# AcrylicShrimp/omok-ai

Hardware: NVIDIA B200
Metric: mcts_simulations_per_sec (higher is better)
Workload: dtype f32

## Files before the change

omok-ai_b200/csrc/omk_api.cu:

```cuda
#include <cstdio>
#include <cstdlib>
#include <cstring>
#include <string>
#include <vector>

#include <utility>

#include "omk_internal.h"

using namespace omk;

static thread_local std::string g_err;
static int32_t fail(int32_t code, const std::string &msg) {
    g_err = msg;
    return code;
}
#define CK(call)                                                                                        \
    do {                                                                                                \
        cudaError_t e__ = (call);                                                                       \
        if (e__ != cudaSuccess)                                                                         \
            return fail(OMK_ERR_CUDA, std::string(#call) + ": " + cudaGetErrorString(e__));             \
    } while (0)
#define CKV(call)                                                                                       \
    do {                                                                                                \
// ... 30 lines not shown
#define SCRATCH(i, count, ptr)                          \
    do {                                                \
        int32_t rc__ = scratch_dev(c, (i), (count), &(ptr)); \
        if (rc__) return rc__;                          \
    } while (0)

static int32_t ensure_workspace(omk_ctx *c, int rows) {
    rows = (rows + 255) / 256 * 256;
    Workspace &w = c->ws;
    if (rows <= w.max_rows) return OMK_OK;
    const size_t r = (size_t)rows;
    w.max_rows = 0;
    CK(w.nn_in.grow(c->stream, r));
    CK(w.req_tree.grow(c->stream, r));
    CK(w.req_node.grow(c->stream, r));
    CK(w.P.grow(c->stream, r * kRow));
    CK(w.V.grow(c->stream, r));
    CK(cudaMemsetAsync(w.nn_in, 0, w.nn_in.bytes(), c->stream));
    w.max_rows = rows;
    return OMK_OK;
}

namespace omk {
bool ensure_activations(omk_ctx *c, int rows) {
    Workspace &w = c->ws;
    rows = (rows + 255) / 256 * 256;
    const bool want_fp32 = c->tower_mode == 0 || c->fc0_mode == 0;
    if (rows <= w.act_rows && (!want_fp32 || w.act_fp32)) return true;
    if (rows < w.act_rows) rows = w.act_rows;
    if (cudaStreamSynchronize(c->stream) != cudaSuccess) return false;
// ... 281 lines not shown
    if (out_h2d) *out_h2d = c->h2d_bytes;
    if (out_d2h) *out_d2h = c->d2h_bytes;
    return OMK_OK;
}

static int32_t sp_refresh_root_policy(omk_ctx *c);

extern "C" int32_t omk_net_load_params(omk_ctx *c, const float *const *tensors, const int64_t *lens) {
    CK(cudaSetDevice(c->device));
    for (int i = 0; i < kNetTensors; ++i)
        if (!tensors[i] || lens[i] != kLens[i])
            return fail(OMK_ERR_INVALID, "tensor " + std::to_string(i) + ": expected " + std::to_string(kLens[i]) + " elements");
    for (int i = 0; i < kNetTensors; ++i)
        CK(copy_h2d(c, c->net.t[i], tensors[i], sizeof(float) * (size_t)kLens[i], c->stream));
    c->net_pack_dirty = false;
    net_pack_heads(c);
    if (!fc16_prepare_weights(c)) return fail(OMK_ERR_CUDA, "fp16-split fc weight preparation failed");
    if (!tower16_prepare_weights(c)) return fail(OMK_ERR_CUDA, "fp16-split tower weight preparation failed");
    CK(cudaStreamSynchronize(c->stream));
    c->net.loaded = true;
    return sp_refresh_root_policy(c);
}
extern "C" int32_t omk_net_get_params(omk_ctx *c, float *const *tensors, const int64_t *lens) {
    CK(cudaSetDevice(c->device));
    if (!c->net.loaded) return fail(OMK_ERR_STATE, "network weights not loaded");
    for (int i = 0; i < kNetTensors; ++i)
        if (!tensors[i] || lens[i] != kLens[i]) return fail(OMK_ERR_INVALID, "bad tensor length");
    for (int i = 0; i < kNetTensors; ++i)
        CK(copy_d2h(c, tensors[i], c->net.t[i], sizeof(float) * (size_t)kLens[i], c->stream));
    CK(cudaStreamSynchronize(c->stream));
    return OMK_OK;
}
extern "C" int32_t omk_net_init_random(omk_ctx *c, uint64_t seed) {
    CK(cudaSetDevice(c->device));
    launch_net_init_random(c, seed);
    c->net_pack_dirty = false;
    net_pack_heads(c);
    if (!fc16_prepare_weights(c)) return fail(OMK_ERR_CUDA, "fp16-split fc weight preparation failed");
    if (!tower16_prepare_weights(c)) return fail(OMK_ERR_CUDA, "fp16-split tower weight preparation failed");
    CK(cudaStreamSynchronize(c->stream));
    CK(cudaGetLastError());
    c->net.loaded = true;
    return sp_refresh_root_policy(c);
}

static int32_t net_eval_common(omk_ctx *c, int n, const float *images_dev, float *out_p, float *out_v, int slot = 0) {
    if (slot == 0) {
        int32_t rc_p = ensure_packed(c);
        if (rc_p) return rc_p;
    }
    ModelScope scope(c, slot);
// ... 35 lines not shown
    CK(cudaSetDevice(c->device));
    if (!c->net.loaded) return fail(OMK_ERR_STATE, "network weights not loaded");
    if (n < 0 || !images || !out_p) return fail(OMK_ERR_INVALID, "bad arguments");
    if (n == 0) return OMK_OK;
    int32_t rc = ensure_workspace(c, n);
    if (rc) return rc;
    float *d_img = nullptr;
    SCRATCH(0, (size_t)n * 243, d_img);
    CK(copy_h2d(c, d_img, images, sizeof(float) * (size_t)n * 243, c->stream));
    const uint32_t nn = (uint32_t)n;
    CK(copy_h2d(c, c->ws.n_req, &nn, sizeof nn, c->stream));
    return net_eval_common(c, n, d_img, out_p, out_v);
}

static int32_t weights_changed(omk_ctx *c) {
    net_pack_heads(c);
    if (!fc16_prepare_weights(c)) return fail(OMK_ERR_CUDA, "fp16-split fc weight preparation failed");
    if (!tower16_prepare_weights(c)) return fail(OMK_ERR_CUDA, "fp16-split tower weight preparation failed");
    CK(cudaStreamSynchronize(c->stream));
    return sp_refresh_root_policy(c);
}

static int32_t train_backward_impl(omk_ctx *c, const float *images, const float *pi, const float *z, int32_t n,
                                   void **out_grads_device, int64_t *out_count, bool sync) {
    CK(cudaSetDevice(c->device));
    if (!c->net.loaded) return fail(OMK_ERR_STATE, "network weights not loaded");
    if (n < 1 || !images || !pi || !z) return fail(OMK_ERR_INVALID, "bad arguments");
    float *g = nullptr;
    c->train_n = 0;
    if (const char *e = train_backward_step(c, images, pi, z, n, &g)) return fail(OMK_ERR_CUDA, std::string("omk_train_backward: ") + e);
// ... 60 lines not shown
extern "C" int32_t omk_train_comm_init(omk_ctx *c, const uint8_t *id, int32_t nranks, int32_t rank) {
    CK(cudaSetDevice(c->device));
    if (!id || nranks < 1 || rank < 0 || rank >= nranks) return fail(OMK_ERR_INVALID, "bad communicator arguments");
    if (const char *e = train_comm_init(c, id, nranks, rank)) return fail(OMK_ERR_STATE, std::string("NCCL: ") + e);
    return OMK_OK;
}
extern "C" int32_t omk_train_comm_destroy(omk_ctx *c) {
    CK(cudaSetDevice(c->device));
    train_comm_destroy(c);
    return OMK_OK;
}

extern "C" int32_t omk_debug_set_fc0_mode(omk_ctx *c, int32_t mode) {
    if (mode != 0 && mode != 1) return fail(OMK_ERR_INVALID, "fc0 mode must be 1 (tcgen05 3xFP16) or 0 (fp32 CUDA cores, A/B check)");
    c->fc0_mode = mode;
    return OMK_OK;
}
extern "C" int32_t omk_debug_set_tower_mode(omk_ctx *c, int32_t mode) {
    if (mode != 0 && mode != 1) return fail(OMK_ERR_INVALID, "tower mode must be 1 (tcgen05 3xFP16) or 0 (fp32 CUDA cores, A/B check)");
    c->tower_mode = mode;
    return OMK_OK;
}
extern "C" int32_t omk_debug_set_fc0_balance(omk_ctx *c, int32_t on) {
    if (on != 0 && on != 1) return fail(OMK_ERR_INVALID, "fc0 balance must be 0 or 1");
    c->fc0_balance = on;
    return OMK_OK;
}
extern "C" int32_t omk_debug_set_fc0_chunk(omk_ctx *c, int32_t k_blocks) {
    if (k_blocks != 3 && k_blocks != 9) return fail(OMK_ERR_INVALID, "fc0 chunk must be 9 (default) or 3 (finer accumulation)");
    CK(cudaStreamSynchronize(c->stream));
    c->fc0_chunk = k_blocks;
    return OMK_OK;
}
extern "C" int32_t omk_debug_set_lane_min_trees(omk_ctx *c, int32_t min_trees) {
    if (min_trees < 0) return fail(OMK_ERR_INVALID, "min_trees < 0");
    c->lane_min_trees = min_trees;
    return OMK_OK;
}
extern "C" int32_t omk_debug_tower_timing(omk_ctx *c, int64_t *out64) {
    CK(cudaSetDevice(c->device));
    CK(cudaStreamSynchronize(c->stream));
    tower16_read_timing(reinterpret_cast<long long *>(out64));
    return OMK_OK;
}
extern "C" int32_t omk_debug_get_buffer(omk_ctx *c, int32_t which, float *out, int64_t count) {
    CK(cudaSetDevice(c->device));
// ... 566 lines not shown
        int8_t *d_status = reinterpret_cast<int8_t *>(ds + slot.off_status);
        for (int l = 0; l < lanes; ++l) {
            LaneScope scope(c, l, 0);
            const int g0 = lane_g0[l], nl = lane_n[l];
            bool sp = span_begin(OMK_K_MOVE);
            launch_sp_prepare(c, g0, nl, mover, other, modes, temps);
            launch_root_noise(c, mover + g0, nl, cfg.epsilon, cfg.alpha);
            span_end(sp);
        }
        for (int r = 0; r < rounds; ++r) {
            for (int l = 0; l < lanes; ++l) {
                LaneScope scope(c, l, 0);
                const int g0 = lane_g0[l], nl = lane_n[l];
                bool sp = span_begin(OMK_K_SELECT);
                launch_reset_requests(c);
                launch_select_expand(c, mover + g0, nl, cfg.batch_size);
                span_end(sp);
                RUN_EVAL(c, cfg.evaluator, nl * cfg.batch_size);
                sp = span_begin(OMK_K_APPLY);
                launch_apply(c, mover + g0, nl, kApplySearch);
                span_end(sp);
            }
        }
        for (int l = 0; l < lanes; ++l) {
            LaneScope scope(c, l, 0);
            const int g0 = lane_g0[l], nl = lane_n[l];
            const size_t row = (size_t)g0;
            bool sp = span_begin(OMK_K_MOVE);
            launch_sample(c, mover + g0, nl, modes + g0, temps + g0, actions + g0, policy_out + (size_t)g0 * kCells, nullptr);
            launch_sp_record(c, nl, mover + g0, actions + g0, policy_out + (size_t)g0 * kCells, d_boards + row * kCells,
                             d_policy + row * kCells, d_actions + row);
            if (feed) {
                CK(cudaStreamWaitEvent(c->stream, c->rp.ev_commit, 0));
                launch_rp_stage(c, g0, nl, d_boards + row * kCells, d_policy + row * kCells);
            }
// ... 665 lines not shown
```

omok-ai_b200/csrc/omk_device.cuh:

```cuda
#pragma once
#include <cstdint>
#include <cuda_runtime.h>

namespace omk {

constexpr int kCells = 81;
constexpr int kSide = 9;
constexpr int kRow = 96;
constexpr uint32_t kNoNode = 0xFFFFu;
constexpr float kF32Eps = 1.1920929e-7f;

constexpr int kInProgress = 0, kDraw = 1, kBlackWin = 2, kWhiteWin = 3;

constexpr int kNodeBytes = 1408;
constexpr int kOffPolicy = 64;
constexpr int kOffEdgeN = 448;
constexpr int kOffEdgeW = 832;
constexpr int kOffChild = 1216;

struct NodeHdr {
    uint32_t black[3], white[3], cmask[3];
    uint32_t parent, action, status, legal, turn, has_policy;
};

struct __align__(16) TreeHdr {
    uint32_t n_nodes;
    uint32_t root_n;
    float root_w;
    float root_p;
    uint32_t rng_counter;
    uint32_t stream;
    uint32_t noise_epoch;
    uint32_t error;
    uint32_t sims_lo, sims_hi;
    uint32_t pad[6];
};
static_assert(sizeof(TreeHdr) == 64, "TreeHdr is 64 bytes");

// ... 13 lines not shown
    return tree_nodes + (size_t)id * kNodeBytes;
}
__device__ __forceinline__ float *node_policy(uint8_t *n) { return reinterpret_cast<float *>(n + kOffPolicy); }
__device__ __forceinline__ uint32_t *node_edge_n(uint8_t *n) { return reinterpret_cast<uint32_t *>(n + kOffEdgeN); }
__device__ __forceinline__ float *node_edge_w(uint8_t *n) { return reinterpret_cast<float *>(n + kOffEdgeW); }
__device__ __forceinline__ uint16_t *node_child(uint8_t *n) { return reinterpret_cast<uint16_t *>(n + kOffChild); }

__device__ __forceinline__ NodeHdr load_hdr(const uint8_t *n) {
    const uint4 *q = reinterpret_cast<const uint4 *>(n);
    const uint4 a = q[0], b = q[1], c = q[2];
    NodeHdr h;
    h.black[0] = a.x; h.black[1] = a.y; h.black[2] = a.z;
    h.white[0] = a.w; h.white[1] = b.x; h.white[2] = b.y;
    h.cmask[0] = b.z; h.cmask[1] = b.w; h.cmask[2] = c.x;
    h.parent = c.y & 0xFFFFu; h.action = (c.y >> 16) & 0xFFu; h.status = c.y >> 24;
    h.legal = c.z & 0xFFu; h.turn = (c.z >> 8) & 0xFFu; h.has_policy = (c.z >> 16) & 0xFFu;
    return h;
}
__device__ __forceinline__ void store_hdr(uint8_t *n, const NodeHdr &h) {
    uint4 *q = reinterpret_cast<uint4 *>(n);
    q[0] = make_uint4(h.black[0], h.black[1], h.black[2], h.white[0]);
    q[1] = make_uint4(h.white[1], h.white[2], h.cmask[0], h.cmask[1]);
    q[2] = make_uint4(h.cmask[2], h.parent | (h.action << 16) | (h.status << 24),
                      h.legal | (h.turn << 8) | (h.has_policy << 16), 0u);
}

__device__ __forceinline__ uint32_t sel3(uint32_t w0, uint32_t w1, uint32_t w2, int word) {
    return word == 0 ? w0 : (word == 1 ? w1 : w2);
}
__device__ __forceinline__ bool bit81(const uint32_t *m, int i) { return (sel3(m[0], m[1], m[2], i >> 5) >> (i & 31)) & 1u; }
__device__ __forceinline__ void set81(uint32_t *m, int i) {
    const uint32_t b = 1u << (i & 31);
    if ((i >> 5) == 0) m[0] |= b; else if ((i >> 5) == 1) m[1] |= b; else m[2] |= b;
}
__device__ __forceinline__ int popc81(const uint32_t *m) { return __popc(m[0]) + __popc(m[1]) + __popc(m[2] & 0x1FFFFu); }
__device__ __forceinline__ int nth_set_bit32(uint32_t w, int r) {
    for (int i = 0; i < r; ++i) w &= w - 1;
    return __ffs(w) - 1;
}
// ... 182 lines not shown
```

omok-ai_b200/csrc/omk_internal.h:

```cpp
#pragma once
#include <cstdint>
#include <memory>
#include <utility>
#include <vector>
#include <cuda.h>
#include <cuda_fp16.h>
#include <cuda_runtime.h>

#include "../../include/omok_b200.h"
#include "omk_device.cuh"

namespace omk {

constexpr int kMaxBatchPerTree = 64;
constexpr int kNetTensors = 31;
constexpr int kModelSlots = 16;

enum ApplyMode { kApplySearch = 0, kApplyNewGame = 1, kApplyEnsure = 2 };

struct DeviceMem {
    static cudaError_t alloc(void **p, size_t bytes) { return cudaMalloc(p, bytes); }
    static void release(void *p) { cudaFree(p); }
};
struct PinnedMem {
// ... 83 lines not shown
    bool act_fp32 = false;
    Buf<__half> act0_h16, act0_l16;
    Buf<__half> act1_h16, act1_l16;
    Buf<__half> act2_h16, act2_l16;
    Buf<float> act2;
    Buf<float> logits;
    Buf<float> act0;
    Buf<float> act1;
    ActMaps maps;
};
struct Workspace : Activations {
    int max_rows = 0;
    Buf<NNIn> nn_in;
    Buf<uint32_t> req_tree;
    Buf<uint32_t> req_node;
    Buf<float> P;
    Buf<float> V;
    Buf<uint32_t> n_req;
    Buf<uint32_t> slot_base, slot_count;
    Buf<int32_t> ids;
    Buf<int32_t> actions;
    Buf<uint8_t> modes;
    Buf<float> temps;
    Buf<int8_t> status;
    Buf<float> policy_out;
    Buf<uint32_t> streams;
    Buf<float> splitk_partial;
    Buf<float4> bal_partial;
    Buf<uint32_t> bal_flags;
};
// ... 73 lines not shown
    omk::NetWeights opp;
    omk::NetWeights more[omk::kModelSlots - 2];
    omk::NetWeights *model = &net;
    omk::NetWeights &slot(int s) { return s == 0 ? net : (s == 1 ? opp : more[s - 2]); }
    omk::Workspace ws;
    int virtual_loss = 0;
    int fc0_balance = 0;
    int fc0_chunk = 9;
    int fc0_mode = 1;
    std::unique_ptr<omk::Fc16State, omk::Fc16StateFree> fc16_state;
    int tower16_pairs = 0;
    std::unique_ptr<omk::TrainState, omk::TrainStateFree> train_state;
    int train_n = 0;
    bool net_pack_dirty = false;
    int tower_mode = 1;

    omk_selfplay_config sp_cfg{};
    bool sp_active = false;
    omk::Buf<int32_t> sp_ply;
    omk::Buf<uint8_t> sp_buf;
    static constexpr int kSpRing = 4;
    omk::Buf<uint8_t> sp_ring_dev;
    omk::PinnedBuf<uint8_t> sp_ring_host;
    size_t sp_ring_slot_bytes = 0;
    cudaStream_t sp_copy_stream = nullptr;
    cudaEvent_t sp_ev_rec[kSpRing][2] = {}, sp_ev_copy[kSpRing] = {};
    omk::Replay rp;
    omk::Buf<uint8_t> eval_buf;
    cudaEvent_t ev0 = nullptr, ev1 = nullptr;
};
// ... 1 lines not shown
namespace omk {

void launch_env_reset(omk_ctx *c, const int32_t *ids_dev, int n);
void launch_env_step(omk_ctx *c, const int32_t *ids_dev, const uint8_t *actions_dev, int n, int8_t *status_dev,
                     uint32_t *legal_dev);
void launch_env_get(omk_ctx *c, const int32_t *ids_dev, int n, uint8_t *boards_dev, uint8_t *turns_dev,
                    uint16_t *legal_dev);
void launch_env_set(omk_ctx *c, const int32_t *ids_dev, int n, const uint8_t *boards_dev, const uint8_t *turns_dev);
void launch_env_encode(omk_ctx *c, const int32_t *ids_dev, int n, int mode, float *out_dev);
void launch_env_playout(omk_ctx *c, int n, int plies, uint8_t *actions_dev, int8_t *status_dev);
void launch_pack_boards(omk_ctx *c, const uint8_t *boards_dev, const uint8_t *turns_dev, int n, int mode);

void launch_new_games(omk_ctx *c, const int32_t *ids_dev, int n, const uint32_t *streams_dev,
                      const int8_t *only_if_terminal, const float *root_policy);
void launch_root_noise(omk_ctx *c, const int32_t *ids_dev, int n, float epsilon, float alpha);
void launch_select_expand(omk_ctx *c, const int32_t *ids_dev, int n, int batch);
void launch_apply(omk_ctx *c, const int32_t *ids_dev, int n, int mode);
void launch_sample(omk_ctx *c, const int32_t *ids_dev, int n, const uint8_t *modes_dev, const float *temps_dev,
                   int32_t *actions_dev, float *policy_dev, uint8_t *valid_dev);
void launch_ensure_prepare(omk_ctx *c, const int32_t *ids_dev, const int32_t *actions_dev, int n);
void launch_play(omk_ctx *c, const int32_t *ids_dev, const int32_t *actions_dev, int n, int8_t *status_dev);
void launch_root_children(omk_ctx *c, int tree, int32_t *actions_dev, unsigned long long *n_dev, float *w_dev,
                          float *p_dev, int32_t *len_dev, float *policy_dev, uint32_t *misc_dev);
void launch_eval_hash(omk_ctx *c, int rows_bound);
void launch_pool_get_envs(omk_ctx *c, const int32_t *ids_dev, int n, uint8_t *boards_dev, uint8_t *turns_dev,
                          uint16_t *legal_dev, int8_t *status_dev);
void launch_reset_requests(omk_ctx *c);
void launch_sp_prepare(omk_ctx *c, int g0, int n, int32_t *mover, int32_t *other, uint8_t *modes, float *temps);
void launch_sp_record(omk_ctx *c, int n, const int32_t *mover, const int32_t *actions, const float *policy_in,
                      uint8_t *boards_out, float *policy_out, int32_t *actions_out);
void launch_sp_advance(omk_ctx *c, int g0, int n, const int8_t *status, unsigned long long *counters);

// ... 65 lines not shown
```

omok-ai_b200/csrc/tree_kernels.cu:

```cuda
#include "omk_internal.h"

namespace omk {

constexpr int kWarpsPerBlock = 4;
constexpr unsigned kFull = 0xffffffffu;

struct TreeArgs {
    TreeHdr *hdrs;
    uint8_t *nodes;
    int cap_nodes;
    const int32_t *ids;
    int id_base;
    int n;
    uint64_t seed;
    uint32_t *dev_error;
    unsigned long long *dev_sims;
    NNIn *nn_in;
    uint32_t *req_tree, *req_node;
    uint32_t *n_req;
    uint32_t *slot_base, *slot_count;
    const float *P, *V;
    int max_rows;
    int vloss;
};

__device__ __forceinline__ int tree_of(const TreeArgs &a, int slot) { return a.ids ? a.ids[slot] : slot + a.id_base; }
__device__ __forceinline__ uint8_t *tree_nodes_of(const TreeArgs &a, int tree) {
    return a.nodes + (size_t)tree * (size_t)a.cap_nodes * kNodeBytes;
}

__device__ __forceinline__ float dummy_prior(const NodeHdr &h, int a) {
    const uint32_t occ = sel3(h.black[0] | h.white[0], h.black[1] | h.white[1], h.black[2] | h.white[2], a >> 5);
    if ((occ >> (a & 31)) & 1u) return 0.0f;
    if (h.legal == 0) return 1.0f;
    return __fmul_rn(1.0f, __fdiv_rn(1.0f, (float)h.legal));
}

__device__ __forceinline__ float seq_sum81(const float v[3]) {
    float s = 0.0f;
#pragma unroll
    for (int j = 0; j < 3; ++j) {
        const int lim = j == 2 ? kCells - 64 : 32;
        for (int l = 0; l < lim; ++l) s = __fadd_rn(s, __shfl_sync(kFull, v[j], l));
// ... 104 lines not shown
        const float inv = __fdiv_rn(1.0f, s);
#pragma unroll
        for (int j = 0; j < 3; ++j) nz[j] = __fmul_rn(nz[j], inv);
        if (lane == 0) th->noise_epoch = epoch + 1;
    }
    const float keep = __fsub_rn(1.0f, epsilon);
#pragma unroll
    for (int j = 0; j < 3; ++j) p[j] = __fadd_rn(__fmul_rn(keep, p[j]), __fmul_rn(epsilon, nz[j]));
    const float s = seq_sum81(p);
    const float inv = __fdiv_rn(1.0f, s);
#pragma unroll
    for (int j = 0; j < 3; ++j) {
        const int c = lane + 32 * j;
        if (c < kCells) pol[c] = __fmul_rn(p[j], inv);
    }
    if (lane == 0 && !h.has_policy) {
        h.has_policy = 1;
        store_hdr(tn, h);
    }
}

__global__ void __launch_bounds__(kWarpsPerBlock * 32) k_select_expand(TreeArgs a, int batch) {
    __shared__ uint32_t s_path[kWarpsPerBlock][kCells + 3];
    __shared__ uint16_t s_req[kWarpsPerBlock][kMaxBatchPerTree];
    const int wib = threadIdx.x >> 5;
    const int slot = blockIdx.x * kWarpsPerBlock + wib;
    const int lane = threadIdx.x & 31;
    if (slot >= a.n) return;
    const int tree = tree_of(a, slot);
    uint8_t *tn = tree_nodes_of(a, tree);
    TreeHdr *th = &a.hdrs[tree];
    uint32_t *path = s_path[wib];
    uint16_t *req = s_req[wib];

    uint32_t n_nodes = th->n_nodes;
    uint32_t root_n = th->root_n;
    float root_w = th->root_w;
    uint32_t rng_counter = th->rng_counter;
    const uint32_t stream = th->stream;
    uint32_t err = th->error;
    uint32_t sims = 0;
    int nreq = 0;

    bool restart = true;
    uint32_t x = 0;
    uint32_t cur_n = root_n;
    int depth = 0;
    NodeHdr h{};
    int it = 0;
    while (it < batch && !err) {
        if (restart) {
            x = 0;
            cur_n = root_n;
            depth = 0;
            h = load_hdr(tn);
            restart = false;
        }
        for (;;) {
            const int nch = popc81(h.cmask);
            if (nch != (int)h.legal || nch == 0) break;
            uint8_t *xn = node_ptr(tn, x);
            const uint32_t parent_n = cur_n > 1u ? cur_n : 1u;
            const float sq = __fsqrt_rn((float)parent_n);
            const uint32_t *en = node_edge_n(xn);
            const float *ew = node_edge_w(xn);
            const float *pol = node_policy(xn);
            const uint16_t *ch = node_child(xn);
            unsigned long long best = 0ull;
            uint32_t best_n = 0;
            int best_a = 0;
// ... 18 lines not shown
            }
            unsigned long long wbest = best;
#pragma unroll
            for (int off = 16; off > 0; off >>= 1) {
                const unsigned long long o = __shfl_xor_sync(kFull, wbest, off);
                wbest = o > wbest ? o : wbest;
            }
            const int src = __ffs(__ballot_sync(kFull, best == wbest && best != 0ull)) - 1;
            best_n = __shfl_sync(kFull, best_n, src);
            best_a = __shfl_sync(kFull, best_a, src);
            if (lane == 0) path[depth] = (x << 8) | (uint32_t)best_a;
            ++depth;
            x = (uint32_t)(wbest & 0xFFFFFFFFull) - 1u;
            cur_n = best_n;
            h = load_hdr(node_ptr(tn, x));
        }
        __syncwarp();

        if (h.status != kInProgress) {
            ++it;
            ++sims;
            if (lane == 0) {
                const float z = (h.status == kBlackWin || h.status == kWhiteWin) ? 1.0f : 0.0f;
                backup_path(tn, path, depth, z, root_n, root_w);
            }
            root_n = __shfl_sync(kFull, root_n, 0);
            root_w = __shfl_sync(kFull, root_w, 0);
            __syncwarp();
            restart = true;
            continue;
// ... 25 lines not shown
            }
        }
        NodeHdr c = h;
        bool five = false;
        if (lane < K) {
            uint32_t *mine = h.turn == 0 ? c.black : c.white;
            set81(mine, my_action);
            five = makes_five_scalar(mine, my_action);
            c.legal = h.legal - 1;
            c.turn = h.turn ^ 1u;
            c.status = five ? (h.turn == 0 ? kBlackWin : kWhiteWin) : (c.legal == 0 ? kDraw : kInProgress);
            c.cmask[0] = c.cmask[1] = c.cmask[2] = 0;
            c.parent = x;
            c.action = (uint32_t)my_action;
            c.has_policy = 0;
        }
        const uint32_t term_mask = __ballot_sync(kFull, lane < K && c.status != kInProgress);
        const int t_first = term_mask ? __ffs(term_mask) - 1 : K;
        int accepted = t_first < K ? t_first + 1 : K;
        if (n_nodes + (uint32_t)accepted > (uint32_t)a.cap_nodes) {
            accepted = (int)((uint32_t)a.cap_nodes - n_nodes);
            err = 1;
        }
        const bool term_accepted = t_first < accepted;
        const uint32_t id = n_nodes + (uint32_t)lane;
        uint8_t *xn = node_ptr(tn, x);
        uint32_t add[3] = {0u, 0u, 0u};
        if (lane < accepted) {
            store_hdr(node_ptr(tn, id), c);
            node_edge_n(xn)[my_action] = 0u;
            node_edge_w(xn)[my_action] = 0.0f;
            node_child(xn)[my_action] = (uint16_t)id;
            add[my_action >> 5] = 1u << (my_action & 31);
            if (lane < t_first) req[nreq + lane] = (uint16_t)id;
        }
#pragma unroll
        for (int k = 0; k < 3; ++k) {
            add[k] = __reduce_or_sync(kFull, add[k]);
            h.cmask[k] |= add[k];
        }
        if (lane < 3 && sel3(add[0], add[1], add[2], lane)) reinterpret_cast<uint32_t *>(xn)[6 + lane] = sel3(h.cmask[0], h.cmask[1], h.cmask[2], lane);
        if (accepted > 0) rng_counter = __shfl_sync(kFull, my_ctr, accepted - 1);
        n_nodes += (uint32_t)accepted;
        nreq += min(t_first, accepted);
        it += accepted;
        sims += (uint32_t)accepted;
        __syncwarp();
        if (term_accepted) {
            const int t_action = __shfl_sync(kFull, my_action, t_first);
// ... 13 lines not shown
                    node_edge_n(pn)[pa] += 1u;
                    node_edge_w(pn)[pa] = __fsub_rn(node_edge_w(pn)[pa], 1.0f);
                }
                root_n += 1u;
            }
            restart = true;
        }
#ifdef OMK_NO_DESCENT_REUSE
        restart = true;
#endif
        root_n = __shfl_sync(kFull, root_n, 0);
        root_w = __shfl_sync(kFull, root_w, 0);
        __syncwarp();
    }

    uint32_t base = 0;
    if (lane == 0) base = nreq ? atomicAdd(a.n_req, (uint32_t)nreq) : 0u;
    base = __shfl_sync(kFull, base, 0);
    if (base + (uint32_t)nreq > (uint32_t)a.max_rows) {
        err = 1;
        nreq = 0;
    }
    __syncwarp();
    for (int i = lane; i < nreq; i += 32) {
        const uint32_t id = req[i];
        const NodeHdr r = load_hdr(node_ptr(tn, id));
        NNIn in;
        in.black[0] = r.black[0]; in.black[1] = r.black[1]; in.black[2] = r.black[2];
        in.white[0] = r.white[0]; in.white[1] = r.white[1]; in.white[2] = r.white[2];
        in.meta = r.turn;
        in.pad = 0;
        a.nn_in[base + i] = in;
        a.req_tree[base + i] = (uint32_t)tree;
        a.req_node[base + i] = id;
    }
    if (lane == 0) {
        a.slot_base[slot] = base;
        a.slot_count[slot] = (uint32_t)nreq;
        th->n_nodes = n_nodes;
        th->root_n = root_n;
        th->root_w = root_w;
        th->rng_counter = rng_counter;
        if (err) {
            th->error = err;
            atomicOr(a.dev_error, 1u);
        }
        atomicAdd(a.dev_sims, (unsigned long long)sims);
    }
}

__global__ void __launch_bounds__(kWarpsPerBlock * 32) k_apply(TreeArgs a, int mode) {
    constexpr int kChunk = 16;
    __shared__ float s_p[kWarpsPerBlock][kChunk][kCells];
    __shared__ uint32_t s_meta[kWarpsPerBlock][kChunk][4];
    const int wib = threadIdx.x >> 5;
    const int slot = blockIdx.x * kWarpsPerBlock + wib;
    const int lane = threadIdx.x & 31;
    if (slot >= a.n) return;
    const int tree = tree_of(a, slot);
    uint8_t *tn = tree_nodes_of(a, tree);
    TreeHdr *th = &a.hdrs[tree];
    const uint32_t base = a.slot_base[slot];
    const int cnt = (int)a.slot_count[slot];
    if (cnt == 0) return;
    uint32_t root_n = th->root_n;
    float root_w = th->root_w;
    uint32_t root_occ[3] = {0u, 0u, 0u};
    if (mode == kApplyEnsure) {
        const NodeHdr root_h = load_hdr(tn);
#pragma unroll
        for (int k = 0; k < 3; ++k) root_occ[k] = root_h.black[k] | root_h.white[k];
    }
    float(*sp)[kCells] = s_p[wib];
    uint32_t(*meta)[4] = s_meta[wib];

    for (int c0 = 0; c0 < cnt; c0 += kChunk) {
        const int m = min(kChunk, cnt - c0);
        const uint32_t row0 = base + (uint32_t)c0;
        uint32_t my_id = 0, my_action = 0;
        float my_v = 0.0f;
        uint32_t my_occ[3] = {0u, 0u, 0u};
        if (lane < m) {
            my_id = a.req_node[row0 + lane];
            if (mode == kApplySearch) my_v = -a.V[row0 + lane];
            const NodeHdr h = load_hdr(node_ptr(tn, my_id));
#pragma unroll
            for (int k = 0; k < 3; ++k) my_occ[k] = h.black[k] | h.white[k];
            my_action = h.action;
            meta[lane][0] = my_id;
            meta[lane][1] = h.parent | (h.action << 16);
            meta[lane][2] = h.legal | (h.turn << 8) | (1u << 16);
            meta[lane][3] = __float_as_uint(my_v);
        }
#pragma unroll 8
        for (int i = 0; i < m; ++i) {
            const float *Prow = a.P + (size_t)(row0 + i) * kRow;
            float pv[3];
#pragma unroll
            for (int j = 0; j < 3; ++j) {
                const int c = lane + 32 * j;
                pv[j] = c < kCells ? Prow[c] : 0.0f;
            }
            const uint32_t o0 = __shfl_sync(kFull, my_occ[0], i), o1 = __shfl_sync(kFull, my_occ[1], i), o2 = __shfl_sync(kFull, my_occ[2], i);
            const int act_i = (int)__shfl_sync(kFull, my_action, i);
#pragma unroll
            for (int j = 0; j < 3; ++j) {
                const int c = lane + 32 * j;
                if (c < kCells) {
                    float v = pv[j];
                    if (mode == kApplySearch) {
                        const uint32_t occ = sel3(o0, o1, o2, j);
                        if ((occ >> (c & 31)) & 1u) v = 0.0f;
                    } else if (mode == kApplyEnsure) {
                        const uint32_t occ = sel3(root_occ[0], root_occ[1], root_occ[2], j);
                        if (c == act_i || ((occ >> (c & 31)) & 1u)) v = 0.0f;
                    }
                    sp[i][c] = v;
                }
            }
        }
        __syncwarp();
        float inv = 0.0f;
        bool scale = false;
        if (mode != kApplyNewGame && lane < m) {
            float sum = 0.0f;
#pragma unroll 9
            for (int c = 0; c < kCells; ++c) sum = __fadd_rn(sum, sp[lane][c]);
            scale = kF32Eps <= sum;
            if (scale) inv = __fdiv_rn(1.0f, sum);
        }
#pragma unroll 4
        for (int i = 0; i < m; ++i) {
            const float inv_i = __shfl_sync(kFull, inv, i);
            const bool scale_i = __shfl_sync(kFull, (int)scale, i) != 0;
            const uint32_t id = __shfl_sync(kFull, my_id, i);
            float *pol = node_policy(node_ptr(tn, id));
#pragma unroll
            for (int j = 0; j < 3; ++j) {
                const int c = lane + 32 * j;
                if (c < kCells) {
                    const float v = sp[i][c];
                    pol[c] = scale_i ? __fmul_rn(v, inv_i) : v;
                }
            }
        }
        if (lane < m) {
            uint8_t *nd = node_ptr(tn, meta[lane][0]);
            reinterpret_cast<uint32_t *>(nd)[10] = meta[lane][2];
            if (mode == kApplySearch) {
                const uint32_t par = meta[lane][1] & 0xFFFFu, act = (meta[lane][1] >> 16) & 0xFFu;
                if (par != kNoNode) {
                    uint8_t *pn = node_ptr(tn, par);
                    const float v = __uint_as_float(meta[lane][3]);
                    if (a.vloss) {
                        node_edge_w(pn)[act] = __fadd_rn(node_edge_w(pn)[act], __fadd_rn(v, 1.0f));
                    } else {
                        node_edge_n(pn)[act] += 1u;
                        node_edge_w(pn)[act] = __fadd_rn(node_edge_w(pn)[act], v);
                    }
                }
            }
        }
        __syncwarp();
// ... 194 lines not shown
    if (action >= 0 && action < kCells) {
        const NodeHdr h = load_hdr(tn);
        if (!bit81(h.cmask, action)) {
            c = h;
            const uint32_t occ = sel3(h.black[0] | h.white[0], h.black[1] | h.white[1], h.black[2] | h.white[2], action >> 5);
            if (!((occ >> (action & 31)) & 1u)) {
                set81(h.turn == 0 ? c.black : c.white, action);
                c.legal = h.legal - 1;
                c.turn = h.turn ^ 1u;
            }
            c.status = kInProgress;
            c.cmask[0] = c.cmask[1] = c.cmask[2] = 0;
            c.parent = 0;
            c.action = (uint32_t)action;
            c.has_policy = 0;
            const uint32_t n_nodes = th->n_nodes;
            if (n_nodes >= (uint32_t)a.cap_nodes) {
                if (lane == 0) {
                    th->error = 1;
                    atomicOr(a.dev_error, 1u);
                }
            } else {
                id = n_nodes;
                nreq = 1;
                if (lane == 0) {
                    th->n_nodes = n_nodes + 1;
                    store_hdr(node_ptr(tn, id), c);
                    reinterpret_cast<uint32_t *>(tn)[6 + (action >> 5)] =
                        sel3(h.cmask[0], h.cmask[1], h.cmask[2], action >> 5) | (1u << (action & 31));
                    node_edge_n(tn)[action] = 0u;
// ... 266 lines not shown
    a.id_base = ids_dev ? 0 : c->id_base;
    a.n = n;
    a.seed = c->seed;
    a.dev_error = c->dev_error;
    a.dev_sims = c->dev_sims;
    a.nn_in = c->ws.nn_in;
    a.req_tree = c->ws.req_tree;
    a.req_node = c->ws.req_node;
    a.n_req = c->ws.n_req;
    a.slot_base = c->ws.slot_base;
    a.slot_count = c->ws.slot_count;
    a.P = c->ws.P;
    a.V = c->ws.V;
    a.max_rows = c->ws.max_rows;
    a.vloss = c->virtual_loss;
    return a;
}
static inline int warp_grid(int n) { return (n + kWarpsPerBlock - 1) / kWarpsPerBlock; }

void launch_reset_requests(omk_ctx *c) {
    k_reset_requests<<<1, 1, 0, c->stream>>>(c->ws.n_req, c->dev_sims);
    c->launches++;
}
void launch_new_games(omk_ctx *c, const int32_t *ids_dev, int n, const uint32_t *streams_dev,
                      const int8_t *only_if_terminal, const float *root_policy) {
    if (n <= 0) return;
    k_new_games<<<warp_grid(n), kWarpsPerBlock * 32, 0, c->stream>>>(make_args(c, ids_dev, n), streams_dev,
                                                                       only_if_terminal, root_policy);
    c->launches++;
}
// ... 4 lines not shown
}
void launch_sp_record(omk_ctx *c, int n, const int32_t *mover, const int32_t *actions, const float *policy_in,
                      uint8_t *boards_out, float *policy_out, int32_t *actions_out) {
    k_sp_record<<<n, 96, 0, c->stream>>>(make_args(c, mover, n), actions, policy_in, boards_out, policy_out, actions_out);
    c->launches++;
}
void launch_sp_advance(omk_ctx *c, int g0, int n, const int8_t *status, unsigned long long *counters) {
    k_sp_advance<<<(n + 127) / 128, 128, 0, c->stream>>>(g0, n, c->sp_ply, status, counters, c->dev_error);
    c->launches++;
}
void launch_root_noise(omk_ctx *c, const int32_t *ids_dev, int n, float epsilon, float alpha) {
    if (n <= 0) return;
    k_root_noise<<<warp_grid(n), kWarpsPerBlock * 32, 0, c->stream>>>(make_args(c, ids_dev, n), epsilon, alpha);
    c->launches++;
}
void launch_select_expand(omk_ctx *c, const int32_t *ids_dev, int n, int batch) {
    if (n <= 0) return;
    k_select_expand<<<warp_grid(n), kWarpsPerBlock * 32, 0, c->stream>>>(make_args(c, ids_dev, n), batch);
    c->launches++;
}
void launch_apply(omk_ctx *c, const int32_t *ids_dev, int n, int mode) {
    if (n <= 0) return;
    k_apply<<<warp_grid(n), kWarpsPerBlock * 32, 0, c->stream>>>(make_args(c, ids_dev, n), mode);
    c->launches++;
}
void launch_sample(omk_ctx *c, const int32_t *ids_dev, int n, const uint8_t *modes_dev, const float *temps_dev,
                   int32_t *actions_dev, float *policy_dev, uint8_t *valid_dev) {
    if (n <= 0) return;
    k_sample<<<warp_grid(n), kWarpsPerBlock * 32, 0, c->stream>>>(make_args(c, ids_dev, n), modes_dev, temps_dev,
                                                                    actions_dev, policy_dev, valid_dev);
    c->launches++;
}
void launch_ensure_prepare(omk_ctx *c, const int32_t *ids_dev, const int32_t *actions_dev, int n) {
    if (n <= 0) return;
    k_ensure_prepare<<<warp_grid(n), kWarpsPerBlock * 32, 0, c->stream>>>(make_args(c, ids_dev, n), actions_dev);
    c->launches++;
}
void launch_play(omk_ctx *c, const int32_t *ids_dev, const int32_t *actions_dev, int n, int8_t *status_dev) {
// ... 29 lines not shown
```

Before: 17.36 million.

## Reuse twin tree's cached NN evaluations to skip duplicate network rows

During self-play search, each tree is paired with its twin (the other player's tree, which sees the same game). When expanding a leaf, the kernel walks the twin tree along the same path. If the twin already holds an evaluated node with the same board, turn and network generation, the cached policy and value are reused and that request is not sent to the network. Only the misses are compacted into the network batch, with a per-request source index stored in a new buffer, and apply reads P and V either from the batch or from the twin node. A net generation counter invalidates the cache on weight or mode changes. The cost is extra header words, twin traversal and more divergent gathers in apply.

Result: faster. 17.54 million, median of 6 (+1.0%).

```diff
diff --git a/omok-ai_b200/csrc/omk_api.cu b/omok-ai_b200/csrc/omk_api.cu
--- a/omok-ai_b200/csrc/omk_api.cu
+++ b/omok-ai_b200/csrc/omk_api.cu
@@ -68,6 +68,7 @@
     CK(w.nn_in.grow(c->stream, r));
     CK(w.req_tree.grow(c->stream, r));
     CK(w.req_node.grow(c->stream, r));
+    CK(w.req_src.grow(c->stream, r));
     CK(w.P.grow(c->stream, r * kRow));
     CK(w.V.grow(c->stream, r));
     CK(cudaMemsetAsync(w.nn_in, 0, w.nn_in.bytes(), c->stream));
@@ -379,6 +380,7 @@
     for (int i = 0; i < kNetTensors; ++i)
         CK(copy_h2d(c, c->net.t[i], tensors[i], sizeof(float) * (size_t)kLens[i], c->stream));
     c->net_pack_dirty = false;
+    ++c->net_gen;
     net_pack_heads(c);
     if (!fc16_prepare_weights(c)) return fail(OMK_ERR_CUDA, "fp16-split fc weight preparation failed");
     if (!tower16_prepare_weights(c)) return fail(OMK_ERR_CUDA, "fp16-split tower weight preparation failed");
@@ -400,6 +402,7 @@
     CK(cudaSetDevice(c->device));
     launch_net_init_random(c, seed);
     c->net_pack_dirty = false;
+    ++c->net_gen;
     net_pack_heads(c);
     if (!fc16_prepare_weights(c)) return fail(OMK_ERR_CUDA, "fp16-split fc weight preparation failed");
     if (!tower16_prepare_weights(c)) return fail(OMK_ERR_CUDA, "fp16-split tower weight preparation failed");
@@ -465,6 +468,7 @@
 }
 
 static int32_t weights_changed(omk_ctx *c) {
+    ++c->net_gen;
     net_pack_heads(c);
     if (!fc16_prepare_weights(c)) return fail(OMK_ERR_CUDA, "fp16-split fc weight preparation failed");
     if (!tower16_prepare_weights(c)) return fail(OMK_ERR_CUDA, "fp16-split tower weight preparation failed");
@@ -555,22 +559,26 @@
 extern "C" int32_t omk_debug_set_fc0_mode(omk_ctx *c, int32_t mode) {
     if (mode != 0 && mode != 1) return fail(OMK_ERR_INVALID, "fc0 mode must be 1 (tcgen05 3xFP16) or 0 (fp32 CUDA cores, A/B check)");
     c->fc0_mode = mode;
+    ++c->net_gen;
     return OMK_OK;
 }
 extern "C" int32_t omk_debug_set_tower_mode(omk_ctx *c, int32_t mode) {
     if (mode != 0 && mode != 1) return fail(OMK_ERR_INVALID, "tower mode must be 1 (tcgen05 3xFP16) or 0 (fp32 CUDA cores, A/B check)");
     c->tower_mode = mode;
+    ++c->net_gen;
     return OMK_OK;
 }
 extern "C" int32_t omk_debug_set_fc0_balance(omk_ctx *c, int32_t on) {
     if (on != 0 && on != 1) return fail(OMK_ERR_INVALID, "fc0 balance must be 0 or 1");
     c->fc0_balance = on;
+    ++c->net_gen;
     return OMK_OK;
 }
 extern "C" int32_t omk_debug_set_fc0_chunk(omk_ctx *c, int32_t k_blocks) {
     if (k_blocks != 3 && k_blocks != 9) return fail(OMK_ERR_INVALID, "fc0 chunk must be 9 (default) or 3 (finer accumulation)");
     CK(cudaStreamSynchronize(c->stream));
     c->fc0_chunk = k_blocks;
+    ++c->net_gen;
     return OMK_OK;
 }
 extern "C" int32_t omk_debug_set_lane_min_trees(omk_ctx *c, int32_t min_trees) {
@@ -1167,11 +1175,11 @@
                 const int g0 = lane_g0[l], nl = lane_n[l];
                 bool sp = span_begin(OMK_K_SELECT);
                 launch_reset_requests(c);
-                launch_select_expand(c, mover + g0, nl, cfg.batch_size);
+                launch_select_expand(c, mover + g0, nl, cfg.batch_size, other + g0);
                 span_end(sp);
                 RUN_EVAL(c, cfg.evaluator, nl * cfg.batch_size);
                 sp = span_begin(OMK_K_APPLY);
-                launch_apply(c, mover + g0, nl, kApplySearch);
+                launch_apply(c, mover + g0, nl, kApplySearch, other + g0);
                 span_end(sp);
             }
         }
diff --git a/omok-ai_b200/csrc/omk_device.cuh b/omok-ai_b200/csrc/omk_device.cuh
--- a/omok-ai_b200/csrc/omk_device.cuh
+++ b/omok-ai_b200/csrc/omk_device.cuh
@@ -21,7 +21,9 @@
 struct NodeHdr {
     uint32_t black[3], white[3], cmask[3];
     uint32_t parent, action, status, legal, turn, has_policy;
-};
+    uint32_t shared;
+};
+constexpr int kHdrWordV = 12, kHdrWordGen = 13;
 
 struct __align__(16) TreeHdr {
     uint32_t n_nodes;
@@ -65,7 +67,7 @@
     h.white[0] = a.w; h.white[1] = b.x; h.white[2] = b.y;
     h.cmask[0] = b.z; h.cmask[1] = b.w; h.cmask[2] = c.x;
     h.parent = c.y & 0xFFFFu; h.action = (c.y >> 16) & 0xFFu; h.status = c.y >> 24;
-    h.legal = c.z & 0xFFu; h.turn = (c.z >> 8) & 0xFFu; h.has_policy = (c.z >> 16) & 0xFFu;
+    h.legal = c.z & 0xFFu; h.turn = (c.z >> 8) & 0xFFu; h.has_policy = (c.z >> 16) & 0xFFu; h.shared = c.z >> 24;
     return h;
 }
 __device__ __forceinline__ void store_hdr(uint8_t *n, const NodeHdr &h) {
@@ -73,7 +75,7 @@
     q[0] = make_uint4(h.black[0], h.black[1], h.black[2], h.white[0]);
     q[1] = make_uint4(h.white[1], h.white[2], h.cmask[0], h.cmask[1]);
     q[2] = make_uint4(h.cmask[2], h.parent | (h.action << 16) | (h.status << 24),
-                      h.legal | (h.turn << 8) | (h.has_policy << 16), 0u);
+                      h.legal | (h.turn << 8) | (h.has_policy << 16) | (h.shared << 24), 0u);
 }
 
 __device__ __forceinline__ uint32_t sel3(uint32_t w0, uint32_t w1, uint32_t w2, int word) {
diff --git a/omok-ai_b200/csrc/omk_internal.h b/omok-ai_b200/csrc/omk_internal.h
--- a/omok-ai_b200/csrc/omk_internal.h
+++ b/omok-ai_b200/csrc/omk_internal.h
@@ -121,6 +121,7 @@
     Buf<NNIn> nn_in;
     Buf<uint32_t> req_tree;
     Buf<uint32_t> req_node;
+    Buf<uint32_t> req_src;
     Buf<float> P;
     Buf<float> V;
     Buf<uint32_t> n_req;
@@ -224,6 +225,7 @@
     int train_n = 0;
     bool net_pack_dirty = false;
     int tower_mode = 1;
+    uint32_t net_gen = 1;
 
     omk_selfplay_config sp_cfg{};
     bool sp_active = false;
@@ -255,8 +257,8 @@
 void launch_new_games(omk_ctx *c, const int32_t *ids_dev, int n, const uint32_t *streams_dev,
                       const int8_t *only_if_terminal, const float *root_policy);
 void launch_root_noise(omk_ctx *c, const int32_t *ids_dev, int n, float epsilon, float alpha);
-void launch_select_expand(omk_ctx *c, const int32_t *ids_dev, int n, int batch);
-void launch_apply(omk_ctx *c, const int32_t *ids_dev, int n, int mode);
+void launch_select_expand(omk_ctx *c, const int32_t *ids_dev, int n, int batch, const int32_t *twin_dev = nullptr);
+void launch_apply(omk_ctx *c, const int32_t *ids_dev, int n, int mode, const int32_t *twin_dev = nullptr);
 void launch_sample(omk_ctx *c, const int32_t *ids_dev, int n, const uint8_t *modes_dev, const float *temps_dev,
                    int32_t *actions_dev, float *policy_dev, uint8_t *valid_dev);
 void launch_ensure_prepare(omk_ctx *c, const int32_t *ids_dev, const int32_t *actions_dev, int n);
diff --git a/omok-ai_b200/csrc/tree_kernels.cu b/omok-ai_b200/csrc/tree_kernels.cu
--- a/omok-ai_b200/csrc/tree_kernels.cu
+++ b/omok-ai_b200/csrc/tree_kernels.cu
@@ -22,11 +22,25 @@
     const float *P, *V;
     int max_rows;
     int vloss;
+    const int32_t *twin;
+    uint32_t *req_src;
+    uint32_t gen;
 };
+constexpr uint32_t kReqHit = 0x80000000u;
 
 __device__ __forceinline__ int tree_of(const TreeArgs &a, int slot) { return a.ids ? a.ids[slot] : slot + a.id_base; }
 __device__ __forceinline__ uint8_t *tree_nodes_of(const TreeArgs &a, int tree) {
     return a.nodes + (size_t)tree * (size_t)a.cap_nodes * kNodeBytes;
+}
+__device__ __forceinline__ uint32_t child_or_none(uint8_t *n, int act) {
+    const uint32_t m = reinterpret_cast<const uint32_t *>(n)[6 + (act >> 5)];
+    return (m >> (act & 31)) & 1u ? (uint32_t)node_child(n)[act] : kNoNode;
+}
+__device__ __forceinline__ bool twin_serves(const uint8_t *t, const NodeHdr &c, uint32_t gen) {
+    const uint4 *q = reinterpret_cast<const uint4 *>(t);
+    const uint4 q0 = q[0], q1 = q[1], q2 = q[2], q3 = q[3];
+    return q0.x == c.black[0] && q0.y == c.black[1] && q0.z == c.black[2] && q0.w == c.white[0] && q1.x == c.white[1] &&
+           q1.y == c.white[2] && ((q2.z >> 8) & 0xFFu) == c.turn && (q2.z >> 24) == 1u && q3.y == gen;
 }
 
 __device__ __forceinline__ float dummy_prior(const NodeHdr &h, int a) {
@@ -161,8 +175,9 @@
         const int c = lane + 32 * j;
         if (c < kCells) pol[c] = __fmul_rn(p[j], inv);
     }
-    if (lane == 0 && !h.has_policy) {
+    if (lane == 0 && (!h.has_policy || h.shared)) {
         h.has_policy = 1;
+        h.shared = 0;
         store_hdr(tn, h);
     }
 }
@@ -170,6 +185,7 @@
 __global__ void __launch_bounds__(kWarpsPerBlock * 32) k_select_expand(TreeArgs a, int batch) {
     __shared__ uint32_t s_path[kWarpsPerBlock][kCells + 3];
     __shared__ uint16_t s_req[kWarpsPerBlock][kMaxBatchPerTree];
+    __shared__ uint16_t s_src[kWarpsPerBlock][kMaxBatchPerTree];
     const int wib = threadIdx.x >> 5;
     const int slot = blockIdx.x * kWarpsPerBlock + wib;
     const int lane = threadIdx.x & 31;
@@ -179,6 +195,9 @@
     TreeHdr *th = &a.hdrs[tree];
     uint32_t *path = s_path[wib];
     uint16_t *req = s_req[wib];
+    uint16_t *src = s_src[wib];
+    uint8_t *twn = a.twin ? tree_nodes_of(a, a.twin[slot]) : nullptr;
+    uint32_t tw = kNoNode;
 
     uint32_t n_nodes = th->n_nodes;
     uint32_t root_n = th->root_n;
@@ -201,6 +220,7 @@
             cur_n = root_n;
             depth = 0;
             h = load_hdr(tn);
+            tw = twn ? 0u : kNoNode;
             restart = false;
         }
         for (;;) {
@@ -249,6 +269,7 @@
             x = (uint32_t)(wbest & 0xFFFFFFFFull) - 1u;
             cur_n = best_n;
             h = load_hdr(node_ptr(tn, x));
+            if (tw != kNoNode) tw = child_or_none(node_ptr(twn, tw), best_a);
         }
         __syncwarp();
 
@@ -304,6 +325,7 @@
             c.parent = x;
             c.action = (uint32_t)my_action;
             c.has_policy = 0;
+            c.shared = 0;
         }
         const uint32_t term_mask = __ballot_sync(kFull, lane < K && c.status != kInProgress);
         const int t_first = term_mask ? __ffs(term_mask) - 1 : K;
@@ -322,7 +344,12 @@
             node_edge_w(xn)[my_action] = 0.0f;
             node_child(xn)[my_action] = (uint16_t)id;
             add[my_action >> 5] = 1u << (my_action & 31);
-            if (lane < t_first) req[nreq + lane] = (uint16_t)id;
+            if (lane < t_first) {
+                req[nreq + lane] = (uint16_t)id;
+                uint32_t t = tw != kNoNode ? child_or_none(node_ptr(twn, tw), my_action) : kNoNode;
+                if (t != kNoNode && !twin_serves(node_ptr(twn, t), c, a.gen)) t = kNoNode;
+                src[nreq + lane] = (uint16_t)t;
+            }
         }
 #pragma unroll
         for (int k = 0; k < 3; ++k) {
@@ -366,28 +393,47 @@
         __syncwarp();
     }
 
+    __syncwarp();
+    int nmiss = nreq;
+    if (twn) {
+        int k = 0;
+        for (int i = lane; i < nreq; i += 32) k += src[i] == kNoNode;
+        nmiss = __reduce_add_sync(kFull, k);
+    }
     uint32_t base = 0;
-    if (lane == 0) base = nreq ? atomicAdd(a.n_req, (uint32_t)nreq) : 0u;
+    if (lane == 0) base = nmiss ? atomicAdd(a.n_req, (uint32_t)nmiss) : 0u;
     base = __shfl_sync(kFull, base, 0);
-    if (base + (uint32_t)nreq > (uint32_t)a.max_rows) {
+    const uint32_t rec0 = twn ? (uint32_t)slot * (uint32_t)batch : base;
+    if (base + (uint32_t)nmiss > (uint32_t)a.max_rows || rec0 + (uint32_t)nreq > (uint32_t)a.max_rows) {
         err = 1;
         nreq = 0;
     }
-    __syncwarp();
-    for (int i = lane; i < nreq; i += 32) {
-        const uint32_t id = req[i];
-        const NodeHdr r = load_hdr(node_ptr(tn, id));
-        NNIn in;
-        in.black[0] = r.black[0]; in.black[1] = r.black[1]; in.black[2] = r.black[2];
-        in.white[0] = r.white[0]; in.white[1] = r.white[1]; in.white[2] = r.white[2];
-        in.meta = r.turn;
-        in.pad = 0;
-        a.nn_in[base + i] = in;
-        a.req_tree[base + i] = (uint32_t)tree;
-        a.req_node[base + i] = id;
+    uint32_t row = base;
+    for (int i0 = 0; i0 < nreq; i0 += 32) {
+        const int i = i0 + lane;
+        const uint32_t id = i < nreq ? req[i] : 0u;
+        const uint32_t t = i < nreq && twn ? src[i] : kNoNode;
+        const bool miss = i < nreq && t == kNoNode;
+        const uint32_t mm = __ballot_sync(kFull, miss);
+        const uint32_t my_row = row + __popc(mm & ((1u << lane) - 1u));
+        row += __popc(mm);
+        if (miss) {
+            const NodeHdr r = load_hdr(node_ptr(tn, id));
+            NNIn in;
+            in.black[0] = r.black[0]; in.black[1] = r.black[1]; in.black[2] = r.black[2];
+            in.white[0] = r.white[0]; in.white[1] = r.white[1]; in.white[2] = r.white[2];
+            in.meta = r.turn;
+            in.pad = 0;
+            a.nn_in[my_row] = in;
+            a.req_tree[my_row] = (uint32_t)tree;
+        }
+        if (i < nreq) {
+            a.req_node[rec0 + i] = id;
+            if (twn) a.req_src[rec0 + i] = miss ? my_row : (kReqHit | t);
+        }
     }
     if (lane == 0) {
-        a.slot_base[slot] = base;
+        a.slot_base[slot] = rec0;
         a.slot_count[slot] = (uint32_t)nreq;
         th->n_nodes = n_nodes;
         th->root_n = root_n;
@@ -411,6 +457,7 @@
     if (slot >= a.n) return;
     const int tree = tree_of(a, slot);
     uint8_t *tn = tree_nodes_of(a, tree);
+    uint8_t *twn = a.twin ? tree_nodes_of(a, a.twin[slot]) : nullptr;
     TreeHdr *th = &a.hdrs[tree];
     const uint32_t base = a.slot_base[slot];
     const int cnt = (int)a.slot_count[slot];
@@ -429,12 +476,21 @@
     for (int c0 = 0; c0 < cnt; c0 += kChunk) {
         const int m = min(kChunk, cnt - c0);
         const uint32_t row0 = base + (uint32_t)c0;
-        uint32_t my_id = 0, my_action = 0;
-        float my_v = 0.0f;
+        uint32_t my_id = 0, my_action = 0, my_src = row0 + lane;
+        float my_v = 0.0f, my_raw = 0.0f;
+        bool my_hit = false;
         uint32_t my_occ[3] = {0u, 0u, 0u};
         if (lane < m) {
             my_id = a.req_node[row0 + lane];
-            if (mode == kApplySearch) my_v = -a.V[row0 + lane];
+            if (twn) {
+                my_src = a.req_src[row0 + lane];
+                my_hit = (my_src & kReqHit) != 0u;
+            }
+            if (mode == kApplySearch) {
+                my_raw = my_hit ? __uint_as_float(reinterpret_cast<const uint32_t *>(node_ptr(twn, my_src & 0xFFFFu))[kHdrWordV])
+                                : a.V[my_src];
+                my_v = -my_raw;
+            }
             const NodeHdr h = load_hdr(node_ptr(tn, my_id));
 #pragma unroll
             for (int k = 0; k < 3; ++k) my_occ[k] = h.black[k] | h.white[k];
@@ -446,7 +502,8 @@
         }
 #pragma unroll 8
         for (int i = 0; i < m; ++i) {
-            const float *Prow = a.P + (size_t)(row0 + i) * kRow;
+            const uint32_t src_i = __shfl_sync(kFull, my_src, i);
+            const float *Prow = (src_i & kReqHit) ? node_policy(node_ptr(twn, src_i & 0xFFFFu)) : a.P + (size_t)src_i * kRow;
             float pv[3];
 #pragma unroll
             for (int j = 0; j < 3; ++j) {
@@ -474,7 +531,7 @@
         __syncwarp();
         float inv = 0.0f;
         bool scale = false;
-        if (mode != kApplyNewGame && lane < m) {
+        if (mode != kApplyNewGame && lane < m && !my_hit) {
             float sum = 0.0f;
 #pragma unroll 9
             for (int c = 0; c < kCells; ++c) sum = __fadd_rn(sum, sp[lane][c]);
@@ -497,8 +554,14 @@
             }
         }
         if (lane < m) {
-            uint8_t *nd = node_ptr(tn, meta[lane][0]);
-            reinterpret_cast<uint32_t *>(nd)[10] = meta[lane][2];
+            uint32_t *nw = reinterpret_cast<uint32_t *>(node_ptr(tn, meta[lane][0]));
+            if (twn) {
+                nw[kHdrWordV] = __float_as_uint(my_raw);
+                nw[kHdrWordGen] = a.gen;
+                nw[10] = meta[lane][2] | (1u << 24);
+            } else {
+                nw[10] = meta[lane][2];
+            }
             if (mode == kApplySearch) {
                 const uint32_t par = meta[lane][1] & 0xFFFFu, act = (meta[lane][1] >> 16) & 0xFFu;
                 if (par != kNoNode) {
@@ -723,6 +786,7 @@
             c.parent = 0;
             c.action = (uint32_t)action;
             c.has_policy = 0;
+            c.shared = 0;
             const uint32_t n_nodes = th->n_nodes;
             if (n_nodes >= (uint32_t)a.cap_nodes) {
                 if (lane == 0) {
@@ -1019,6 +1083,8 @@
     a.V = c->ws.V;
     a.max_rows = c->ws.max_rows;
     a.vloss = c->virtual_loss;
+    a.req_src = c->ws.req_src;
+    a.gen = c->net_gen;
     return a;
 }
 static inline int warp_grid(int n) { return (n + kWarpsPerBlock - 1) / kWarpsPerBlock; }
@@ -1053,14 +1119,18 @@
     k_root_noise<<<warp_grid(n), kWarpsPerBlock * 32, 0, c->stream>>>(make_args(c, ids_dev, n), epsilon, alpha);
     c->launches++;
 }
-void launch_select_expand(omk_ctx *c, const int32_t *ids_dev, int n, int batch) {
+void launch_select_expand(omk_ctx *c, const int32_t *ids_dev, int n, int batch, const int32_t *twin_dev) {
     if (n <= 0) return;
-    k_select_expand<<<warp_grid(n), kWarpsPerBlock * 32, 0, c->stream>>>(make_args(c, ids_dev, n), batch);
-    c->launches++;
-}
-void launch_apply(omk_ctx *c, const int32_t *ids_dev, int n, int mode) {
+    TreeArgs a = make_args(c, ids_dev, n);
+    a.twin = twin_dev;
+    k_select_expand<<<warp_grid(n), kWarpsPerBlock * 32, 0, c->stream>>>(a, batch);
+    c->launches++;
+}
+void launch_apply(omk_ctx *c, const int32_t *ids_dev, int n, int mode, const int32_t *twin_dev) {
     if (n <= 0) return;
-    k_apply<<<warp_grid(n), kWarpsPerBlock * 32, 0, c->stream>>>(make_args(c, ids_dev, n), mode);
+    TreeArgs a = make_args(c, ids_dev, n);
+    a.twin = mode == kApplySearch ? twin_dev : nullptr;
+    k_apply<<<warp_grid(n), kWarpsPerBlock * 32, 0, c->stream>>>(a, mode);
     c->launches++;
 }
 void launch_sample(omk_ctx *c, const int32_t *ids_dev, int n, const uint8_t *modes_dev, const float *temps_dev,
```
